# Lightbrite88/Argon_Monte_Carlo

Measured on AMD Instinct MI355X. Metric: particle-steps/sec, higher is better.
Workload: dtype f64; 1 GPU; cube_1e5; geometry=cube, n_particles=100000, n_per_gpu=100000, parallelism=single GPU

## Files before the change

argon_monte_carlo_amd/csrc/amc_clusters.hip:

```cpp
#include <stdlib.h>

#define RS_WAVE_SYNC_LDS_ONLY 1
#include "amc_resolve_dev.h"

#define CW_MAXM 16
#define CW_MAXC 24
#define CW_ITEMS 192
#define CW_BLOCKS 512
#define CW_WPB 1

AMC_DEV int cw_adj_head(const amc_resolve_ws &W, unsigned int epoch, int p)
{
    const unsigned long long v = amc_g(W.adj_head)[p];
    return ((unsigned int)(v >> 32) == epoch) ? (int)(unsigned int)(v & 0xffffffffULL) : -1;
}

#define CW_ITERS 3
#define CW_PULLS 4

AMC_DEV void cw_init_slot(const amc_resolve_ws &W, int s, int p, int label, int gen, bool fresh = false)
{
    amc_g(W.slot_of)[p] = s; amc_g(W.sl_moved)[s] = 0;
    auto *m = amc_g((unsigned long long *)&W.sl_meta[s]);
    __hip_atomic_store(m + 0, ((unsigned long long)(unsigned int)label << 32) | (unsigned int)p, __ATOMIC_RELAXED, __HIP_MEMORY_SCOPE_AGENT);
    __hip_atomic_store(m + 1, (unsigned long long)(unsigned int)gen, __ATOMIC_RELAXED, __HIP_MEMORY_SCOPE_AGENT);
    if (!fresh) atomicAnd(&W.sl_hits[s], 0);
}

AMC_DEV double4 cw_load_hist(const amc_resolve_ws &W, int h)
{
    const auto *d = amc_g((const double *)&W.hist[h]);
    double4 r;
    r.x = __hip_atomic_load(d + 0, __ATOMIC_RELAXED, __HIP_MEMORY_SCOPE_AGENT);
    r.y = __hip_atomic_load(d + 1, __ATOMIC_RELAXED, __HIP_MEMORY_SCOPE_AGENT);
    r.z = __hip_atomic_load(d + 2, __ATOMIC_RELAXED, __HIP_MEMORY_SCOPE_AGENT);
    r.w = __hip_atomic_load(d + 3, __ATOMIC_RELAXED, __HIP_MEMORY_SCOPE_AGENT);
    return r;
}

struct cw_lds {
    int mem[64][CW_MAXM];
    int msl[64][CW_MAXM];
    int cnd[64][CW_MAXC];
    int pull[64][CW_PULLS], psl[64][CW_PULLS];
    int nm[64], nc[64], lab[64], npull[64];
    int it0[64];
    int used[64];
    int redo[64];
    int gen[64];
    cw_item item[CW_ITEMS];
    int next[CW_ITEMS];
    int nitems;
    int unv[64];
    double pool_d[10][CW_MAXM];
    int pool_tmp[CW_MAXM], pool_pidx[CW_MAXM], pool_slot[CW_MAXM];
    uint8_t pool_flag[CW_MAXM], pool_moved[CW_MAXM];
};

AMC_DEV void cw_probe_grid(const rs_args &A, rs_shared *wc, cw_lds &L, const cw_item &me, int cell, int s_off)
{
    const amc_resolve_ws &W = A.W;
    const int own = me.own, nm = L.nm[own], lab = L.lab[own];
    const double x = me.x, y = me.y, z = me.z;
    int q = amc_list_head(A.B, cell);
    while (q >= 0) {
        const amc_rec r = amc_g_load(&A.B.rec[q]);
        const int idx = amc_node_particle(A.B, q);
        q = amc_rec_next(r);
        double rx, ry, rz;
        amc_rec_pos(A.G, r, rx, ry, rz);
        const double ax = rx - x, ay = ry - y, az = rz - z;
        if (!(ax * ax + ay * ay + az * az < A.G.cr2_probe)) continue;
        bool mine = false;
        for (int m = 0; m < nm; m++) mine |= L.mem[own][m] == idx;
        if (mine) continue;
        if (cw_adj_head(W, A.sweep_epoch, idx) < 0) {
            const int tag = -(lab + 2);
            const int old = amc_atomic_cas(amc_g(W.slot_of) + idx, -1, tag);
            if (old == tag) continue;
            if (old == -1) {
                const int s = s_off + rs_count_add(&amc_g(wc)->nslots, 1);
                const int k = atomicAdd(&L.npull[own], 1);
                amc_g(W.victim)[idx] = A.sweep_epoch;
                if (s < W.max_slots && k < CW_PULLS) {
                    L.pull[own][k] = idx; L.psl[own][k] = s;
                    L.redo[own] = 1;
                    continue;
                }
                if (s >= W.max_slots) { amc_g(wc)->ovf = 1; rs_raise(W); }
                else { amc_g_store(&W.sl_meta[s], make_int4(idx, s, 0, 0)); amc_g(W.sl_moved)[s] = 0; amc_atomic_and(amc_g(W.sl_hits) + s, 0); }
                amc_g(W.slot_of)[idx] = s < W.max_slots ? s : -1;
            }
        }
        rs_add_edge(W, wc, me.p, idx);
    }
}

AMC_DEV void cw_probe_overlay(const rs_args &A, rs_shared *wc, cw_lds &L, const cw_item &me, int cell, double cr2i, int h_off)
{
    const amc_resolve_ws &W = A.W;
    const int own = me.own, nm = L.nm[own];
    const double x = me.x, y = me.y, z = me.z;
    auto skip_own = [&](int h2) {
        for (int steps = 0; h2 >= 0 && h2 < h_off && steps < CW_ITEMS; steps++) {
            const int c = h2 >> 2, second = (h2 >> 1) & 1, ncs = L.nc[own];
            int t = -1;
            for (int q = 0; q < ncs; q++)
                if (L.cnd[own][q] == c) { t = L.it0[own] + 2 * (q + second * ncs) + (h2 & 1); break; }
            if (t < 0 || t >= CW_ITEMS || L.item[t].h != h2) break;
            h2 = L.next[t];
        }
        return h2;
    };
    int h2 = skip_own(__hip_atomic_load(amc_g(W.ov_head) + cell, __ATOMIC_RELAXED, __HIP_MEMORY_SCOPE_AGENT));
    int guard = 0;
    while (h2 >= 0) {
        if (++guard > W.max_hist) { amc_g(wc)->ovf = 1; rs_raise(W); break; }
        const double4 o = cw_load_hist(W, h2);
        const int nx = __hip_atomic_load(amc_g(W.ov_next) + h2, __ATOMIC_RELAXED, __HIP_MEMORY_SCOPE_AGENT);
        h2 = skip_own(nx);
        const double ax = o.x - x, ay = o.y - y, az = o.z - z;
        if (!(ax * ax + ay * ay + az * az < cr2i)) continue;
        const int s2 = rs_hist_slot(o);
        bool mine = false;
        for (int m = 0; m < nm; m++) mine |= L.msl[own][m] == s2;
        if (mine) continue;
        if (rs_hist_gen(o) != __hip_atomic_load(amc_g((int *)&W.sl_meta[s2]) + 2, __ATOMIC_RELAXED, __HIP_MEMORY_SCOPE_AGENT)) continue;
        rs_add_edge(W, wc, me.p, -(s2 + 2));
    }
}

AMC_DEV int cw_prepare(const amc_resolve_ws &W, rs_shared *wc, cw_lds &L, int own, int h_off)
{
    int m = L.nm[own];
    const int lab = L.lab[own];
    const int np = L.npull[own] < CW_PULLS ? L.npull[own] : CW_PULLS;
    L.unv[own] = 0;
    for (int e = 0; e < np; e++) {
        const int v = L.pull[own][e], sv = L.psl[own][e];
        if (m == CW_MAXM) {
            cw_init_slot(W, sv, v, lab, 0);
            L.unv[own] = 2;
            continue;
        }
        int b = m - 1;
        while (b >= 0 && L.mem[own][b] > v) { L.mem[own][b + 1] = L.mem[own][b]; L.msl[own][b + 1] = L.msl[own][b]; b--; }
        L.mem[own][b + 1] = v; L.msl[own][b + 1] = sv;
        m++;
    }
    L.nm[own] = m; L.npull[own] = 0;
    L.used[own] = 0;
    L.it0[own] = -1;
    return m;
}

AMC_DEV void cw_wide_hooks(rs_wide &wd, cw_lds &L, int own, int h_off)
{
    const int g = L.gen[own];
    wd.cnd = L.cnd[own]; wd.ncnd = L.nc[own];
    wd.used = &L.used[own]; wd.h_off = h_off;
    wd.items = L.item; wd.nitems = &L.nitems; wd.cap = CW_ITEMS;
    wd.own = own; wd.gen = g + 1; wd.it0 = &L.it0[own]; wd.unval = &L.unv[own];
}

AMC_DEV void cw_candidate_slots(const amc_resolve_ws &W, cw_lds &L, int own, int e)
{
    const int c = L.cnd[own][e], m = L.nm[own];
    const int4 cc = amc_g_load(&W.cand4[c]);
    int ai = 0, aj = 0;
    for (int t = 0; t < m; t++) { if (L.mem[own][t] == cc.x) ai = t; if (L.mem[own][t] == cc.y) aj = t; }
    amc_g_store(&W.cand_s[c], make_int4(L.msl[own][ai], L.msl[own][aj], 1, 0));
}

template <int GEOM, bool DBG>
__global__ __launch_bounds__(64 * CW_WPB) void k_clusters_wide(rs_args A_in_kernarg)
{
    long long *const dbg__ = DBG ? A_in_kernarg.dbg : nullptr;
    const long long t_enter__ = dbg__ ? wall_clock64() : 0;
    __shared__ rs_args s_args;
    constexpr int ARG_WORDS = (int)(sizeof(rs_args) / 4), ARG_T = 64 * CW_WPB, ARG_TRIPS = (ARG_WORDS + ARG_T - 1) / ARG_T;
    const int *arg_src = (const int *)__builtin_amdgcn_kernarg_segment_ptr();
    int arg_w[ARG_TRIPS];
#pragma unroll
    for (int j = 0; j < ARG_TRIPS; j++) {
        const int i = (int)threadIdx.x + j * ARG_T;
        arg_w[j] = arg_src[i < ARG_WORDS ? i : ARG_WORDS - 1];
    }
    const int lane = threadIdx.x & 63;
    const int nwaves = gridDim.x * CW_WPB;
    const int wave_id = blockIdx.x * CW_WPB + (threadIdx.x >> 6);
    const int per = A_in_kernarg.wide_per;
    const int k_first = wave_id * per + lane;
    int4 c4_first = make_int4(0, 0, -1, -1);
    unsigned long long mark_first = 0;
    if (lane < per && k_first < A_in_kernarg.W.max_cand) {
        c4_first = A_in_kernarg.W.cand4[k_first]; mark_first = A_in_kernarg.W.cand_mark[k_first];
    }
    int ncand = (int)__hip_atomic_load(&A_in_kernarg.O.cnt->cand_count, __ATOMIC_RELAXED, __HIP_MEMORY_SCOPE_AGENT);
    const int stalled = A_in_kernarg.od_stall ? *A_in_kernarg.od_stall : 0;
#pragma unroll
    for (int j = 0; j < ARG_TRIPS; j++) {
        const int i = (int)threadIdx.x + j * ARG_T;
        if (i < ARG_WORDS) ((int *)&s_args)[i] = arg_w[j];
    }
    __syncthreads();
    const rs_args &A = s_args;
    const amc_resolve_ws &W = A.W;
    rs_shared *wc = (rs_shared *)W.wctl;
    __shared__ cw_lds L_all[CW_WPB];
    cw_lds &L = L_all[threadIdx.x >> 6];
    if (stalled && A.od_tick > stalled) return;
    if (ncand > W.max_cand) ncand = W.max_cand;
    if (wave_id == 0 && lane == 0) {
        amc_g(wc)->active = 1; amc_g(wc)->ncand = ncand;
        if (A.od_done) *amc_g(A.od_done) = A.od_tick;
    }
    if (ncand == 0) return;
    const int s_off = 2 * ncand;
    const int h_off = 4 * ncand;
    const double cr2i = A.P.collision_range * A.P.collision_range * AMC_CR2_INFLATE;
    rs_work K;
    K.x = L.pool_d[0]; K.y = L.pool_d[1]; K.z = L.pool_d[2]; K.vx = L.pool_d[3]; K.vy = L.pool_d[4]; K.vz = L.pool_d[5];
    K.d = L.pool_d[6]; K.dx = L.pool_d[7]; K.dy = L.pool_d[8]; K.dz = L.pool_d[9];
    K.tmp = L.pool_tmp; K.pidx = L.pool_pidx; K.slot = L.pool_slot; K.flag = L.pool_flag; K.moved = L.pool_moved;

    long long t_last = t_enter__;
    long long t_acc[12] = {0, 0, 0, 0, 0, 0, 0, 0, 0, 0, 0, 0};
#define CW_STAMP(slot)                                                                     \
    do {                                                                                   \
        if (timed__) {                                                                     \
            const long long now__ = wall_clock64();                                        \
            t_acc[slot] += now__ - t_last;                                                 \
            t_last = now__;                                                                \
        }                                                                                  \
    } while (0)
    const bool timed__ = DBG && dbg__ && lane == 0 && wave_id * per < ncand;
    if (DBG && dbg__) { asm volatile("s_waitcnt vmcnt(0)" ::: "memory"); CW_STAMP(7); }
    int cat__ = 0;
    long long d_cont = 0, d_three = 0, d_t_load = 0, d_t_emu = 0;
    for (int k0 = wave_id * per; k0 < ncand; k0 += nwaves * per) {
        const int k = k0 + lane;
        const bool valid = lane < per && k < ncand;
        if (lane == 0) L.nitems = 0;
        int4 c4 = make_int4(0, 0, -1, -1);
        int head_i = -1, head_j = -1;
        amc_particle pre_j, pre_i;
        bool fh_ok = false;
        int fh_it0 = -1, fh_pj = -1, fh_pi = -1, fh_sj = -1, fh_si = -1;
        bool iso = false;
        int k2 = -1;
        int4 c4b = make_int4(0, 0, -1, -1);
        unsigned long long mkb = 0;
        if (valid) {
            c4 = (k == k_first) ? c4_first : amc_g_load(&W.cand4[k]);
            const unsigned long long mk = (k == k_first) ? mark_first : amc_g(W.cand_mark)[k];
            const bool marked = (unsigned int)(mk >> 32) == A.sweep_epoch;
            iso = c4.z < 0 && c4.w < 0 && !marked;
            if (c4.z < 0 && c4.w < 0 && marked) {
                const unsigned int succ = (unsigned int)(mk & 0xffffffffULL);
                if (succ != AMC_MARK_MULTI && (int)succ > k && (int)succ < ncand) k2 = (int)succ;
            }
            if (k2 >= 0) { c4b = amc_g_load(&W.cand4[k2]); mkb = amc_g(W.cand_mark)[k2]; }
            else if (!iso) {
                head_i = cw_adj_head(W, A.sweep_epoch, c4.x);
                head_j = cw_adj_head(W, A.sweep_epoch, c4.y);
            }
        }
        CW_STAMP(9);
        if (valid) {
            pre_j = rs_load_particle(A.S, c4.y);
            pre_i = rs_load_particle(A.S, c4.x);
        }
        if (DBG && dbg__) { asm volatile("s_waitcnt vmcnt(0)" ::: "memory"); CW_STAMP(8); }
        CW_STAMP(0);
        bool owner = valid && !iso;
        int nm = 2, nc = 1;
        int *mem = L.mem[lane], *cnd = L.cnd[lane];
        mem[0] = c4.y; mem[1] = c4.x; cnd[0] = k;
        bool chain2 = false;
        if (k2 >= 0) {
            const bool via_x = c4b.z == k && c4b.w < 0, via_y = c4b.w == k && c4b.z < 0;
            chain2 = (unsigned int)(mkb >> 32) != A.sweep_epoch && (via_x || via_y);
            if (chain2) { mem[2] = via_x ? c4b.y : c4b.x; cnd[1] = k2; nm = 3; nc = 2; }
            else {
                head_i = cw_adj_head(W, A.sweep_epoch, c4.x);
                head_j = cw_adj_head(W, A.sweep_epoch, c4.y);
            }
        }
        if (owner && !chain2) {
            for (int cur = 0; cur < nm && owner; cur++) {
                const int p = mem[cur];
                int c = cur == 0 ? head_j : (cur == 1 ? head_i : cw_adj_head(W, A.sweep_epoch, p));
                while (c >= 0) {
                    if (c < k) { owner = false; break; }
                    const int4 r = (c == k) ? c4 : amc_g_load(&W.cand4[c]);
                    const int q = (r.x == p) ? r.y : r.x;
                    const int nx = (r.x == p) ? r.z : r.w;
                    bool seen = false;
                    for (int e = 0; e < nc; e++) seen |= cnd[e] == c;
                    if (!seen) {
                        if (nc == CW_MAXC) { owner = false; amc_g(wc)->changed = 1; rs_raise(W); break; }
                        cnd[nc++] = c;
                    }
                    seen = false;
                    for (int e = 0; e < nm; e++) seen |= mem[e] == q;
                    if (!seen) {
                        if (nm == CW_MAXM) { owner = false; amc_g(wc)->changed = 1; rs_raise(W); break; }
                        mem[nm++] = q;
                    }
                    c = nx;
                }
            }
        }
        if (owner)
            for (int a = 1; a < nm; a++) {
                const int v = mem[a];
                int b = a - 1;
                while (b >= 0 && mem[b] > v) { mem[b + 1] = mem[b]; b--; }
                mem[b + 1] = v;
            }
        CW_STAMP(1);
        const bool take = iso || owner;
        L.nm[lane] = nm; L.nc[lane] = nc; L.lab[lane] = 2 * k; L.npull[lane] = 0;
        for (int m = 0; m < nm; m++) L.msl[lane][m] = 2 * cnd[m >> 1] + (m & 1);
        L.it0[lane] = -1;
        L.redo[lane] = take ? 1 : 0;
        L.gen[lane] = 0;
        if (timed__) cat__ = !take ? 3 : (nm == 2 ? 0 : (nm == 3 ? 1 : 2));
        {
            const int ncl = __popcll(__ballot(take));
            if (lane == 0 && ncl) amc_atomic_add(amc_g(W.wctl) + 32 + (wave_id & 15), ncl);
        }
        rs_wave_sync();
        CW_STAMP(2);
        int first_item = 0;
        for (int iter = 0; iter < CW_ITERS; iter++) {
            rs_wave_sync();
            int my_m = 0;
            if (L.redo[lane]) my_m = cw_prepare(W, wc, L, lane, h_off);
            if (L.redo[lane] && my_m <= 3) {
                const int g = L.gen[lane], lab = L.lab[lane];
                rs_wide wd;
                cw_wide_hooks(wd, L, lane, h_off);
                if (my_m == 2) {
                    const int pj = mem[0], pi = mem[1], sj = L.msl[lane][0], si = L.msl[lane][1];
                    cw_init_slot(W, sj, pj, lab, g + 1, true);
                    cw_init_slot(W, si, pi, lab, g + 1, true);
                    amc_g_store(&W.cand_s[k], make_int4(si, sj, 1, 0));
                    CW_STAMP(11);
                    amc_particle p1 = pre_j, p2 = pre_i;
                    const bool mv = rs_emulate_pair_io<GEOM>(A, wc, p1, p2, pj, pi, sj, si, &wd);
                    fh_ok = mv && L.used[lane] == 1 && !L.unv[lane] && GEOM != AMC_GEOM_CELL;
                    fh_pj = pj; fh_pi = pi; fh_sj = sj; fh_si = si;
                    fh_it0 = L.it0[lane];
                    CW_STAMP(4);
                    L.gen[lane] = g + 1;
                } else {
                    const bool cont = fh_ok && g == 1;
                    fh_ok = false;
                    const long long d_t0 = timed__ ? wall_clock64() : 0;
                    amc_particle q[3];
                    int pidx[3], slot[3];
                    bool moved[3] = {false, false, false};
#pragma unroll
                    for (int a = 0; a < 3; a++) {
                        pidx[a] = mem[a]; slot[a] = L.msl[lane][a];
                        if (g == 0 && pidx[a] == c4.y) q[a] = pre_j;
                        else if (g == 0 && pidx[a] == c4.x) q[a] = pre_i;
                        else q[a] = rs_load_particle(A.S, pidx[a]);
                    }
                    rs_first_hit fh;
                    fh.pj = cont ? fh_pj : -1; fh.pi = cont ? fh_pi : -1;
                    if (cont) { fh.p1 = rs_load_slot(W, fh_sj); fh.p2 = rs_load_slot(W, fh_si); }
                    else { fh.p1 = q[0]; fh.p2 = q[0]; }
                    const int tag = cont ? g : g + 1;
#pragma unroll
                    for (int a = 0; a < 3; a++)
                        if (!cont || (pidx[a] != fh_pj && pidx[a] != fh_pi)) cw_init_slot(W, slot[a], pidx[a], lab, tag);
                    if (cont) { wd.gen = tag; L.used[lane] = 1; L.it0[lane] = fh_it0; }
                    if (g == 0)
                        for (int e = 0; e < L.nc[lane]; e++) cw_candidate_slots(W, L, lane, e);
                    long long d_t1 = 0;
                    if (DBG && timed__) { asm volatile("s_waitcnt vmcnt(0)" ::: "memory"); d_t1 = wall_clock64(); }
                    rs_emulate_small<GEOM, 3>(A, wc, q, pidx, slot, moved, &wd, cont, fh);
                    if (DBG && timed__) { d_three++; d_cont += cont; d_t_load += d_t1 - d_t0; d_t_emu += wall_clock64() - d_t1; }
#pragma unroll
                    for (int a = 0; a < 3; a++)
                        if (moved[a]) rs_store_slot(W, slot[a], q[a]);
                    L.gen[lane] = tag;
                }
                if (L.unv[lane]) rs_add_edge(W, wc, mem[0], mem[0]);
                L.redo[lane] = 0;
            }
            CW_STAMP(3);
            rs_wave_sync();
            unsigned long long todo = __ballot(L.redo[lane] != 0);
            while (todo) {
                const int src = __ffsll((long long)todo) - 1;
                todo &= todo - 1;
                const int g = L.gen[src], ncs = L.nc[src], lab = L.lab[src];
                const int m = L.nm[src];
                if (lane < m) {
                    const int p = L.mem[src][lane], sl = L.msl[src][lane];
                    const amc_particle q = rs_load_particle(A.S, p);
                    rs_store_work(K, lane, q);
                    K.moved[lane] = 0; K.pidx[lane] = p; K.slot[lane] = sl;
                    cw_init_slot(W, sl, p, lab, g + 1);
                }
                if (g == 0)
                    for (int e = lane; e < ncs; e += 64) cw_candidate_slots(W, L, src, e);
                rs_wave_sync();
                rs_wide wd;
                cw_wide_hooks(wd, L, src, h_off);
                if (m <= RS_COOP_MAX) rs_emulate_coop(A, wc, K, 0, m, &wd);
                else if (lane == 0) rs_emulate_generic(A, wc, K, 0, m, &wd);
                rs_wave_sync();
                if (lane < m && K.moved[lane]) rs_store_slot(W, K.slot[lane], rs_load_work(K, lane));
                if (lane == 0) {
                    if (L.unv[src]) rs_add_edge(W, wc, K.pidx[0], K.pidx[0]);
                    L.gen[src] = g + 1;
                    L.redo[src] = 0;
                }
                rs_wave_sync();
            }
            CW_STAMP(4);
            rs_wave_sync();
            const int nit = L.nitems < CW_ITEMS ? L.nitems : CW_ITEMS;
            {
                const int nnew = nit - first_item;
                const int lpi = nnew <= 8 ? 8 : (nnew <= 16 ? 4 : (nnew <= 32 ? 2 : 1));
                const int sub = lane % lpi;
                for (int t = first_item + lane / lpi; t < nit; t += 64 / lpi) {
                    const cw_item it = L.item[t];
                    if (it.pad & 1) continue;
                    for (int c = sub; c < 8; c += lpi) {
                        const int cell = amc_grid_box_cell<true>(A.G, it.x, it.y, it.z, A.G.cr_probe, c);
                        if (cell >= 0) cw_probe_grid(A, wc, L, it, cell, s_off);
                    }
                }
            }
            first_item = nit;
            CW_STAMP(6);
            if (!__ballot(L.redo[lane] != 0)) break;
            if (timed__ && L.redo[0]) cat__ |= 4;
            if (iter + 1 == CW_ITERS || L.nitems >= CW_ITEMS - 8) {
                if (L.redo[lane]) {
                    const int np = L.npull[lane] < CW_PULLS ? L.npull[lane] : CW_PULLS;
                    for (int e = 0; e < np; e++) cw_init_slot(W, L.psl[lane][e], L.pull[lane][e], L.lab[lane], 0);
                    rs_add_edge(W, wc, L.mem[lane][0], L.mem[lane][0]);
                    L.redo[lane] = 0;
                }
                break;
            }
        }
        rs_wave_sync();
        asm volatile("s_waitcnt vmcnt(0)" ::: "memory");
        const int nit = L.nitems < CW_ITEMS ? L.nitems : CW_ITEMS;
        for (int t0 = 0; t0 < nit; t0 += 64) {
            const int t = t0 + lane;
            if (t < nit) L.next[t] = -1;
            if (t < nit) {
                const cw_item it = L.item[t];
                if (!(it.pad & 1) && (it.pad >> 1) == L.gen[it.own]) {
                    int cx, cy, cz;
                    amc_grid_coords(A.G, it.x, it.y, it.z, cx, cy, cz);
                    const int cell = amc_grid_cell<true>(A.G, cx, cy, cz, nullptr);
                    int expected = -1;
                    for (;;) {
                        const int old = amc_atomic_cas(amc_g(W.ov_head) + cell, expected, it.h);
                        if (old == expected) break;
                        expected = old;
                        __hip_atomic_store(amc_g(W.ov_next) + it.h, old, __ATOMIC_RELAXED, __HIP_MEMORY_SCOPE_AGENT);
                        asm volatile("s_waitcnt vmcnt(0)" ::: "memory");
                    }
                    L.next[t] = expected;
                }
            }
        }
        asm volatile("s_waitcnt vmcnt(0)" ::: "memory");
        rs_wave_sync();
        CW_STAMP(5);
        {
            const int lpi = nit <= 8 ? 8 : (nit <= 16 ? 4 : (nit <= 32 ? 2 : 1));
            const int sub = lane % lpi;
            for (int t = lane / lpi; t < nit; t += 64 / lpi) {
                const cw_item it = L.item[t];
                if ((it.pad & 1) || (it.pad >> 1) != L.gen[it.own]) continue;
                for (int c = sub; c < 8; c += lpi) {
                    const int cell = amc_grid_box_cell<true>(A.G, it.x, it.y, it.z, A.G.cr_probe, c);
                    if (cell >= 0) cw_probe_overlay(A, wc, L, it, cell, cr2i, h_off);
                }
            }
        }
        rs_wave_sync();
        CW_STAMP(10);
    }
    if (timed__) {
        long long *R = dbg__ + 128 + 128 * (long long)wave_id;
        const long long t_exit = wall_clock64(), life = t_exit - t_enter__;
        R[0] = t_enter__; R[1] = t_exit; R[2] = A.sweep_epoch;
        R[3] += 1;
        if (life > R[4]) R[4] = life;
        R[5] += d_three; R[6] += d_cont; R[7] += d_t_load; R[124] += d_t_emu;
        R[8 + cat__] += life; R[16 + cat__] += 1;
        for (int e = 0; e < 12; e++) R[32 + 12 * cat__ + e] += t_acc[e];
        if (cat__ == 0) { int bk = (int)(life / 250); if (bk > 7) bk = 7; R[24 + bk] += 1; }
    }
}

int amc_clusters_wide_blocks(amc_ctx *c)
{
    const int nb_env = c->cw_blocks_env;
    if (nb_env > 0) return (nb_env + CW_WPB - 1) / CW_WPB * CW_WPB;
    return CW_BLOCKS;
}

hipError_t amc_launch_clusters_wide(amc_ctx *c, const rs_args &A)
{
    const int nb = amc_clusters_wide_blocks(c);
    const dim3 grid((nb + CW_WPB - 1) / CW_WPB), block(64 * CW_WPB);
    const bool cube = c->P.geometry == AMC_GEOM_CUBE;
    if (A.dbg) {
        if (cube) AMC_LAUNCH(c, (k_clusters_wide<AMC_GEOM_CUBE, true>), grid, block, A);
        else AMC_LAUNCH(c, (k_clusters_wide<AMC_GEOM_PORE, true>), grid, block, A);
    } else {
        if (cube) AMC_LAUNCH(c, (k_clusters_wide<AMC_GEOM_CUBE, false>), grid, block, A);
        else AMC_LAUNCH(c, (k_clusters_wide<AMC_GEOM_PORE, false>), grid, block, A);
    }
    return hipGetLastError();
}
```

Measured before the change: 2.422 billion particle-steps/s.

## Fuse overlay publish and probe into grid probe pass for early-settled clusters

For clusters whose first emulation settles early, items are published into the overlay lists and probed against both grid and overlay within the same first probe pass. This skips the separate publish and overlay sweep for those items. The grid probe now prefetches the next linked-list record and loads list heads one cell per lane. First-hit continuation state moves from registers into LDS and slot indices derived from the candidate. Candidate loads are also hoisted. The change adds extra wave syncs inside the probe loop and complicates the correctness invariants around publication ordering.

```diff
diff --git a/argon_monte_carlo_amd/csrc/amc_clusters.hip b/argon_monte_carlo_amd/csrc/amc_clusters.hip
--- a/argon_monte_carlo_amd/csrc/amc_clusters.hip
+++ b/argon_monte_carlo_amd/csrc/amc_clusters.hip
@@ -51,22 +51,25 @@
     cw_item item[CW_ITEMS];
     int next[CW_ITEMS];
     int nitems;
+    int pub;
     int unv[64];
+    int early[64];
     double pool_d[10][CW_MAXM];
     int pool_tmp[CW_MAXM], pool_pidx[CW_MAXM], pool_slot[CW_MAXM];
     uint8_t pool_flag[CW_MAXM], pool_moved[CW_MAXM];
 };
 
-AMC_DEV void cw_probe_grid(const rs_args &A, rs_shared *wc, cw_lds &L, const cw_item &me, int cell, int s_off)
+AMC_DEV void cw_probe_grid(const rs_args &A, rs_shared *wc, cw_lds &L, const cw_item &me, int q, const amc_rec &r0, int s_off)
 {
     const amc_resolve_ws &W = A.W;
     const int own = me.own, nm = L.nm[own], lab = L.lab[own];
     const double x = me.x, y = me.y, z = me.z;
-    int q = amc_list_head(A.B, cell);
+    amc_rec nx = r0;
     while (q >= 0) {
-        const amc_rec r = amc_g_load(&A.B.rec[q]);
+        const amc_rec r = nx;
         const int idx = amc_node_particle(A.B, q);
         q = amc_rec_next(r);
+        if (q >= 0) nx = amc_g_load(&A.B.rec[q]);
         double rx, ry, rz;
         amc_rec_pos(A.G, r, rx, ry, rz);
         const double ax = rx - x, ay = ry - y, az = rz - z;
@@ -96,8 +99,9 @@
     }
 }
 
-AMC_DEV void cw_probe_overlay(const rs_args &A, rs_shared *wc, cw_lds &L, const cw_item &me, int cell, double cr2i, int h_off)
-{
+AMC_DEV void cw_probe_overlay(const rs_args &A, rs_shared *wc, cw_lds &L, const cw_item &me, int head, int h_off)
+{
+    const double cr2i = A.P.collision_range * A.P.collision_range * AMC_CR2_INFLATE;
     const amc_resolve_ws &W = A.W;
     const int own = me.own, nm = L.nm[own];
     const double x = me.x, y = me.y, z = me.z;
@@ -112,7 +116,7 @@
         }
         return h2;
     };
-    int h2 = skip_own(__hip_atomic_load(amc_g(W.ov_head) + cell, __ATOMIC_RELAXED, __HIP_MEMORY_SCOPE_AGENT));
+    int h2 = skip_own(head);
     int guard = 0;
     while (h2 >= 0) {
         if (++guard > W.max_hist) { amc_g(wc)->ovf = 1; rs_raise(W); break; }
@@ -150,7 +154,7 @@
     }
     L.nm[own] = m; L.npull[own] = 0;
     L.used[own] = 0;
-    L.it0[own] = -1;
+    if (!L.early[own]) L.it0[own] = -1;
     return m;
 }
 
@@ -218,7 +222,6 @@
     if (ncand == 0) return;
     const int s_off = 2 * ncand;
     const int h_off = 4 * ncand;
-    const double cr2i = A.P.collision_range * A.P.collision_range * AMC_CR2_INFLATE;
     rs_work K;
     K.x = L.pool_d[0]; K.y = L.pool_d[1]; K.z = L.pool_d[2]; K.vx = L.pool_d[3]; K.vy = L.pool_d[4]; K.vz = L.pool_d[5];
     K.d = L.pool_d[6]; K.dx = L.pool_d[7]; K.dy = L.pool_d[8]; K.dz = L.pool_d[9];
@@ -241,19 +244,17 @@
     for (int k0 = wave_id * per; k0 < ncand; k0 += nwaves * per) {
         const int k = k0 + lane;
         const bool valid = lane < per && k < ncand;
-        if (lane == 0) L.nitems = 0;
-        int4 c4 = make_int4(0, 0, -1, -1);
+        if (lane == 0) { L.nitems = 0; L.pub = 0; }
+        if (k0 != wave_id * per && valid) { c4_first = amc_g_load(&W.cand4[k]); mark_first = amc_g(W.cand_mark)[k]; }
+        const int4 c4 = valid ? c4_first : make_int4(0, 0, -1, -1);
         int head_i = -1, head_j = -1;
         amc_particle pre_j, pre_i;
-        bool fh_ok = false;
-        int fh_it0 = -1, fh_pj = -1, fh_pi = -1, fh_sj = -1, fh_si = -1;
         bool iso = false;
         int k2 = -1;
         int4 c4b = make_int4(0, 0, -1, -1);
         unsigned long long mkb = 0;
         if (valid) {
-            c4 = (k == k_first) ? c4_first : amc_g_load(&W.cand4[k]);
-            const unsigned long long mk = (k == k_first) ? mark_first : amc_g(W.cand_mark)[k];
+            const unsigned long long mk = mark_first;
             const bool marked = (unsigned int)(mk >> 32) == A.sweep_epoch;
             iso = c4.z < 0 && c4.w < 0 && !marked;
             if (c4.z < 0 && c4.w < 0 && marked) {
@@ -326,6 +327,7 @@
         L.it0[lane] = -1;
         L.redo[lane] = take ? 1 : 0;
         L.gen[lane] = 0;
+        L.early[lane] = 0;
         if (timed__) cat__ = !take ? 3 : (nm == 2 ? 0 : (nm == 3 ? 1 : 2));
         {
             const int ncl = __popcll(__ballot(take));
@@ -350,14 +352,11 @@
                     CW_STAMP(11);
                     amc_particle p1 = pre_j, p2 = pre_i;
                     const bool mv = rs_emulate_pair_io<GEOM>(A, wc, p1, p2, pj, pi, sj, si, &wd);
-                    fh_ok = mv && L.used[lane] == 1 && !L.unv[lane] && GEOM != AMC_GEOM_CELL;
-                    fh_pj = pj; fh_pi = pi; fh_sj = sj; fh_si = si;
-                    fh_it0 = L.it0[lane];
+                    L.early[lane] = mv && L.used[lane] == 1 && !L.unv[lane] && GEOM != AMC_GEOM_CELL;
                     CW_STAMP(4);
                     L.gen[lane] = g + 1;
                 } else {
-                    const bool cont = fh_ok && g == 1;
-                    fh_ok = false;
+                    const bool cont = L.early[lane] && g == 1;
                     const long long d_t0 = timed__ ? wall_clock64() : 0;
                     amc_particle q[3];
                     int pidx[3], slot[3];
@@ -370,14 +369,15 @@
                         else q[a] = rs_load_particle(A.S, pidx[a]);
                     }
                     rs_first_hit fh;
+                    const int fh_pj = c4.y, fh_pi = c4.x;
                     fh.pj = cont ? fh_pj : -1; fh.pi = cont ? fh_pi : -1;
-                    if (cont) { fh.p1 = rs_load_slot(W, fh_sj); fh.p2 = rs_load_slot(W, fh_si); }
+                    if (cont) { fh.p1 = rs_load_slot(W, 2 * k); fh.p2 = rs_load_slot(W, 2 * k + 1); }
                     else { fh.p1 = q[0]; fh.p2 = q[0]; }
                     const int tag = cont ? g : g + 1;
 #pragma unroll
                     for (int a = 0; a < 3; a++)
                         if (!cont || (pidx[a] != fh_pj && pidx[a] != fh_pi)) cw_init_slot(W, slot[a], pidx[a], lab, tag);
-                    if (cont) { wd.gen = tag; L.used[lane] = 1; L.it0[lane] = fh_it0; }
+                    if (cont) { wd.gen = tag; L.used[lane] = 1; }
                     if (g == 0)
                         for (int e = 0; e < L.nc[lane]; e++) cw_candidate_slots(W, L, lane, e);
                     long long d_t1 = 0;
@@ -388,6 +388,7 @@
                     for (int a = 0; a < 3; a++)
                         if (moved[a]) rs_store_slot(W, slot[a], q[a]);
                     L.gen[lane] = tag;
+                    if (g == 0 && !L.unv[lane]) L.early[lane] = 1;
                 }
                 if (L.unv[lane]) rs_add_edge(W, wc, mem[0], mem[0]);
                 L.redo[lane] = 0;
@@ -426,42 +427,76 @@
             CW_STAMP(4);
             rs_wave_sync();
             const int nit = L.nitems < CW_ITEMS ? L.nitems : CW_ITEMS;
-            {
-                const int nnew = nit - first_item;
-                const int lpi = nnew <= 8 ? 8 : (nnew <= 16 ? 4 : (nnew <= 32 ? 2 : 1));
-                const int sub = lane % lpi;
-                for (int t = first_item + lane / lpi; t < nit; t += 64 / lpi) {
-                    const cw_item it = L.item[t];
-                    if (it.pad & 1) continue;
-                    for (int c = sub; c < 8; c += lpi) {
-                        const int cell = amc_grid_box_cell<true>(A.G, it.x, it.y, it.z, A.G.cr_probe, c);
-                        if (cell >= 0) cw_probe_grid(A, wc, L, it, cell, s_off);
+            if (iter == 0 && __ballot(L.early[lane] != 0)) {
+                asm volatile("s_waitcnt vmcnt(0)" ::: "memory");
+                if (lane == 0) L.pub = nit;
+                rs_wave_sync();
+            }
+            const int pub = __builtin_amdgcn_readfirstlane(L.pub);
+            for (int base = first_item; base < nit; base += 8) {
+                int ln = lane;
+                asm volatile("" : "+v"(ln));
+                const int t = base + (ln >> 3), c = ln & 7;
+                const cw_item it = L.item[t < nit ? t : nit - 1];
+                const bool act = t < nit && !(it.pad & 1);
+                const bool one_pass = act && t < pub && L.early[it.own];
+                const int cell = act ? amc_grid_box_cell<true>(A.G, it.x, it.y, it.z, A.G.cr_probe, c) : -1;
+                const unsigned long long gh = amc_g(A.B.head)[cell >= 0 ? cell : 0];
+                int home = -2;
+                if (one_pass) {
+                    int cx, cy, cz;
+                    amc_grid_coords(A.G, it.x, it.y, it.z, cx, cy, cz);
+                    home = amc_grid_cell<true>(A.G, cx, cy, cz, nullptr);
+                }
+                if (cell == home) {
+                    int expected = -1;
+                    for (;;) {
+                        const int old = amc_atomic_cas(amc_g(W.ov_head) + cell, expected, it.h);
+                        if (old == expected) break;
+                        expected = old;
+                        __hip_atomic_store(amc_g(W.ov_next) + it.h, old, __ATOMIC_RELAXED, __HIP_MEMORY_SCOPE_AGENT);
+                        asm volatile("s_waitcnt vmcnt(0)" ::: "memory");
                     }
-                }
+                    L.next[t] = expected;
+                }
+                if (first_item < pub) {
+                    asm volatile("s_waitcnt vmcnt(0)" ::: "memory");
+                    rs_wave_sync();
+                    CW_STAMP(5);
+                }
+                if (cell >= 0) {
+                    const int q = ((unsigned int)(gh >> 32) == A.B.epoch) ? (int)(unsigned int)(gh & 0xffffffffULL) : -1;
+                    const amc_rec r0 = amc_g_load(&A.B.rec[q >= 0 ? q : 0]);
+                    const int ovh = __hip_atomic_load(amc_g(W.ov_head) + cell, __ATOMIC_RELAXED, __HIP_MEMORY_SCOPE_AGENT);
+                    cw_probe_grid(A, wc, L, it, q, r0, s_off);
+                    if (one_pass) cw_probe_overlay(A, wc, L, it, ovh, h_off);
+                }
+                if (first_item < pub) { rs_wave_sync(); CW_STAMP(10); }
             }
             first_item = nit;
             CW_STAMP(6);
             if (!__ballot(L.redo[lane] != 0)) break;
             if (timed__ && L.redo[0]) cat__ |= 4;
-            if (iter + 1 == CW_ITERS || L.nitems >= CW_ITEMS - 8) {
-                if (L.redo[lane]) {
-                    const int np = L.npull[lane] < CW_PULLS ? L.npull[lane] : CW_PULLS;
-                    for (int e = 0; e < np; e++) cw_init_slot(W, L.psl[lane][e], L.pull[lane][e], L.lab[lane], 0);
-                    rs_add_edge(W, wc, L.mem[lane][0], L.mem[lane][0]);
-                    L.redo[lane] = 0;
-                }
-                break;
-            }
+            const bool goes_on = L.nm[lane] == 2 && L.npull[lane] == 1;
+            if (L.redo[lane] && (iter + 1 == CW_ITERS || L.nitems >= CW_ITEMS - 8 || (L.early[lane] && !goes_on))) {
+                const int np = L.npull[lane] < CW_PULLS ? L.npull[lane] : CW_PULLS;
+                for (int e = 0; e < np; e++) cw_init_slot(W, L.psl[lane][e], L.pull[lane][e], L.lab[lane], 0);
+                rs_add_edge(W, wc, L.mem[lane][0], L.mem[lane][0]);
+                L.redo[lane] = 0;
+            }
+            if (iter + 1 == CW_ITERS || L.nitems >= CW_ITEMS - 8 || !__ballot(L.redo[lane] != 0)) break;
         }
         rs_wave_sync();
+        const int nit = L.nitems < CW_ITEMS ? L.nitems : CW_ITEMS;
+        if (nit <= L.pub && !__ballot(L.gen[lane] > 0 && !L.early[lane])) continue;
         asm volatile("s_waitcnt vmcnt(0)" ::: "memory");
-        const int nit = L.nitems < CW_ITEMS ? L.nitems : CW_ITEMS;
         for (int t0 = 0; t0 < nit; t0 += 64) {
             const int t = t0 + lane;
-            if (t < nit) L.next[t] = -1;
             if (t < nit) {
                 const cw_item it = L.item[t];
-                if (!(it.pad & 1) && (it.pad >> 1) == L.gen[it.own]) {
+                const bool done = t < L.pub && L.early[it.own];
+                if (!done) L.next[t] = -1;
+                if (!done && !(it.pad & 1) && (it.pad >> 1) == L.gen[it.own]) {
                     int cx, cy, cz;
                     amc_grid_coords(A.G, it.x, it.y, it.z, cx, cy, cz);
                     const int cell = amc_grid_cell<true>(A.G, cx, cy, cz, nullptr);
@@ -485,10 +520,12 @@
             const int sub = lane % lpi;
             for (int t = lane / lpi; t < nit; t += 64 / lpi) {
                 const cw_item it = L.item[t];
-                if ((it.pad & 1) || (it.pad >> 1) != L.gen[it.own]) continue;
+                if ((it.pad & 1) || (it.pad >> 1) != L.gen[it.own] || (t < L.pub && L.early[it.own])) continue;
                 for (int c = sub; c < 8; c += lpi) {
                     const int cell = amc_grid_box_cell<true>(A.G, it.x, it.y, it.z, A.G.cr_probe, c);
-                    if (cell >= 0) cw_probe_overlay(A, wc, L, it, cell, cr2i, h_off);
+                    if (cell >= 0)
+                        cw_probe_overlay(A, wc, L, it, __hip_atomic_load(amc_g(W.ov_head) + cell, __ATOMIC_RELAXED, __HIP_MEMORY_SCOPE_AGENT),
+                                         h_off);
                 }
             }
         }
```

After: 2.390 billion particle-steps/s. 0.987x the previous value.
